# louisaslett/PhaseType

Measured on NVIDIA B200. Metric: path_draws_per_sec, higher is better.
Workload: dtype f64

## Files before the change

### phasetype_b200/csrc/k_mhrs.cu

```cuda
#include <cooperative_groups.h>
#include "engine_internal.h"
#include "pht_philox.h"

namespace cg = cooperative_groups;

#ifndef MHRS_THREADS
#define MHRS_THREADS 256
#endif
#define MHRS_WARPS (MHRS_THREADS / 32)
#ifndef MHRS_MIN_BLOCKS
#define MHRS_MIN_BLOCKS 4
#endif
#ifndef MHRS_TAIL_MIN_BLOCKS
#define MHRS_TAIL_MIN_BLOCKS 3
#endif
#ifndef MHRS_NOINLINE_COLD
#define MHRS_COLD static __device__ __forceinline__
#else
#define MHRS_COLD static __device__ __noinline__
#endif
#define GUIDE_BITS 8
#define GUIDE (1 << GUIDE_BITS)
#ifndef END_CAP
#define END_CAP 32u
#endif
#ifndef MHRS_REPLAY_MIN_BLOCKS
#define MHRS_REPLAY_MIN_BLOCKS 4
#endif
#ifndef REPLAY_REFILL_MIN
#define REPLAY_REFILL_MIN 16
#endif
#ifndef EV_MIN
#define EV_MIN 8u
#endif
#ifndef EV_WAIT
#define EV_WAIT 16u
#endif
#ifndef PREFETCH_MIN
#define PREFETCH_MIN 8
#endif
#ifndef TAIL_CH
#define TAIL_CH 256u
#endif
#ifndef TAIL_BATCH
#define TAIL_BATCH 1u
#endif
#ifndef TAIL_LATE_P
#define TAIL_LATE_P 1024u
#endif
#ifndef TAIL_LATE_GROWTH
#define TAIL_LATE_GROWTH 4u
#endif
#ifndef DRAIN_LANES
#define DRAIN_LANES 32
#endif
#ifndef TAIL_K0
#define TAIL_K0 512u
#endif
#define TAIL_KMAX (1u << 24)
#ifndef TAIL_GROWTH
#define TAIL_GROWTH 2u
#endif
#ifndef FOUND_PERIOD
#define FOUND_PERIOD 8u
#endif
#define POOL_MIN 32u
#ifndef POOL_MAX
#define POOL_MAX 256u
#endif
#define FOUND_NONE 0xFFFFFFFFFFFFFFFFull
#define T52_NEVER (1ull << 52)
#define LOWBITS (1u << 20)
#define XBAR_TIMEOUT_NS 4000000000ull

#define RF_PROP 2u
#define RF_OFF 4u
#define RF_SKIP 8u

template <int NC>
struct MhrsSmem {
    static constexpr int R = NC + 1;
    unsigned long long thr[R * R];
    double cum[R * R];
    double scale[NC];
    double s[NC];
    double inv_smax;
    unsigned long long zlo[NC];
    long long zhi[NC];
    unsigned int Nacc[NC * NC];
    unsigned int Bacc[NC];
    float A[R + 3];
    unsigned int paths_done;
    unsigned int scan[MHRS_WARPS + 1];
    uint32_t pctr[MHRS_WARPS];
    float pf_yf[MHRS_THREADS]; uint32_t pf_og[MHRS_THREADS], pf_pos[MHRS_THREADS];
    uint32_t mh_cur_a[MHRS_THREADS], mh_misc[MHRS_THREADS];
    unsigned char guide[R * GUIDE];
};

__device__ __forceinline__ unsigned long long gtimer() {
    unsigned long long t; asm volatile("mov.u64 %0, %globaltimer;" : "=l"(t)); return t;
}
__device__ __forceinline__ float lg2_approx(float x) {
    float r; asm("lg2.approx.ftz.f32 %0, %1;" : "=f"(r) : "f"(x)); return r;
}

__device__ __forceinline__ pht_u32x4 philox_block(uint32_t c0, uint32_t c1, uint32_t c2, uint32_t c3, const SweepParams &p) {
    PHT_PHILOX_ROUND(p.rk.k[0], p.rk.k[1])   PHT_PHILOX_ROUND(p.rk.k[2], p.rk.k[3])   PHT_PHILOX_ROUND(p.rk.k[4], p.rk.k[5])
    PHT_PHILOX_ROUND(p.rk.k[6], p.rk.k[7])   PHT_PHILOX_ROUND(p.rk.k[8], p.rk.k[9])   PHT_PHILOX_ROUND(p.rk.k[10], p.rk.k[11])
    PHT_PHILOX_ROUND(p.rk.k[12], p.rk.k[13]) PHT_PHILOX_ROUND(p.rk.k[14], p.rk.k[15]) PHT_PHILOX_ROUND(p.rk.k[16], p.rk.k[17])
    PHT_PHILOX_ROUND(p.rk.k[18], p.rk.k[19])
    pht_u32x4 out; out.v[0] = c0; out.v[1] = c1; out.v[2] = c2; out.v[3] = c3;
    return out;
}

struct Walk {
    double t, spare;
    uint32_t spare_hi, a, b;
    int j;
    bool odd, fresh;
};
struct Rec { double lastt; int B; long out_idx; double *z2; };

__device__ __forceinline__ void walk_begin(Walk &w, uint32_t a, bool off, uint32_t og, const SweepParams &p, uint32_t iter) {
    w.a = a; w.fresh = true; w.b = 0; w.odd = false; w.t = 0.0; w.j = 0; w.spare = 0.0; w.spare_hi = 0u;
    if (off) {
        pht_u32x4 r = philox_block(0u, a, og, iter, p);
        w.spare = pht_u01(r.v[2], r.v[3]); w.spare_hi = r.v[3]; w.odd = true; w.b = 1;
    }
}

__device__ __forceinline__ double log_unit(double x) { return pht_log_core(pht_d2u(x), 0); }

template <bool RECORD, int NC>
__device__ __forceinline__ bool walk_step(Walk &w, double y, bool cens, uint32_t og, const SweepParams &p, MhrsSmem<NC> &sm,
                                          uint32_t iter, int n, Rec &rec) {
    constexpr int R = NC + 1;
    pht_u32x4 r = philox_block(w.b, w.a, og, iter, p);
    w.b++;
    const double f = pht_u01(r.v[0], r.v[1]), g = pht_u01(r.v[2], r.v[3]);
    const double uA = w.odd ? w.spare : f;
    const uint32_t hiA = w.odd ? w.spare_hi : r.v[1];
    const double uB = w.odd ? f : g;
    w.spare = g; w.spare_hi = r.v[3];
    const bool fresh = w.fresh;
    const int row = fresh ? n : w.j;
    const int last = fresh ? n - 1 : n;
    const double *c = sm.cum + row * R;
    int k = sm.guide[row * GUIDE + (hiA >> (32 - GUIDE_BITS))] & 0x7f;
    while (k < last && c[k] < uA) k++;
    const bool cont = (k < n) && (w.t < y || cens);
    const bool ended = !fresh && !cont;
    const bool advance = !fresh && cont;
    if (RECORD) {
        if (advance) {
            rec.z2[w.j] += w.t - rec.lastt;
            if (p.outN != nullptr) p.outN[(size_t)rec.out_idx * n * n + w.j + k * n]++;
            else atomicAdd(&sm.Nacc[w.j + k * n], 1u);
        }
        rec.lastt = fresh ? 0.0 : (advance ? w.t : rec.lastt);
        rec.B = fresh ? k : rec.B;
    }
    const double tb = fresh ? 0.0 : w.t;
    const int jn = ended ? w.j : k;
    const double tn = tb + sm.scale[jn] * (-log_unit(uB));
    w.t = ended ? w.t : tn;
    w.j = jn;
    w.fresh = false;
    return ended;
}

template <int NC, bool IV = false>
MHRS_COLD uint32_t exact_attempt(uint32_t a, bool off, double y, bool cens, uint32_t og, const SweepParams &p,
                                                      MhrsSmem<NC> &sm, uint32_t iter, int n, uint32_t smask, double u = 0.0) {
    Walk w; Rec norec; norec.lastt = 0.0; norec.B = 0; norec.out_idx = 0; norec.z2 = nullptr;
    walk_begin(w, a, off, og, p, iter);
    unsigned st = 1;
    while (!walk_step<false>(w, y, cens, og, p, sm, iter, n, norec)) st++;
    bool ok = (w.t >= y) && ((smask >> w.j) & 1u);
    if constexpr (IV) ok = ok && w.t <= u;
// ... 143 lines not shown
    f.row = absd ? f.row : k;
    return end;
}

template <bool IV>
__device__ __forceinline__ bool fast_survives(const Fast &f, const typename ObsOf<IV>::T &o) {
    bool s = f.t - o.yn > f.dacc;
    if constexpr (IV) s = s && -(f.t - o.un) > f.dacc;
    return s;
}

template <int NC>
__device__ __forceinline__ void build_tables(const SweepParams &p, MhrsSmem<NC> &sm, int n, const ModelLayout &ML) {
    constexpr int R = NC + 1;
    const int tid = threadIdx.x;
    double smax = 0.0;
    for (int i = 0; i < n; i++) { const double sc = p.model[ML.scale + i]; smax = (sc > smax) ? sc : smax; }
    const double inv_smax = 1.0 / smax;
    for (int i = tid; i < n; i += MHRS_THREADS) {
        const double sc = p.model[ML.scale + i];
        sm.scale[i] = sc; sm.s[i] = p.model[ML.s + i]; sm.zlo[i] = 0ull; sm.zhi[i] = 0; sm.Bacc[i] = 0u;
        sm.A[i] = (float)((-0.69314718055994530942 * sc) * inv_smax);
    }
    if (tid == 0) { sm.A[n] = 0.0f; sm.inv_smax = inv_smax; }
    for (int i = tid; i < n * n; i += MHRS_THREADS) sm.Nacc[i] = 0u;
    for (int e = tid; e < R * R; e += MHRS_THREADS) {
        const int row = e / R, k = e % R;
        unsigned long long t52 = T52_NEVER; double c = 0.0;
        if (row <= n && k <= n) {
            c = p.model[ML.cum + row * (n + 1) + k];
            const int last = (row == n) ? n - 1 : n;
            if (k < last && c < 1.0) {
                if (!(c > 0.0)) t52 = 0ull;
                else {
                    const unsigned long long xf = (unsigned long long)(c * 4503599627370496.0);
                    const double u = pht_u2d(0x3ff0000000000000ULL | xf) - 0.99999999999999988898;
                    t52 = (u > c) ? xf : xf + 1ull;
                }
            }
        }
        sm.thr[e] = t52; sm.cum[e] = c;
    }
    if (tid == 0) sm.paths_done = 0u;
    __syncthreads();
    for (int e = tid; e < (n + 1) * GUIDE; e += MHRS_THREADS) {
        const int row = e / GUIDE, b = e % GUIDE, last = (row == n) ? n - 1 : n;
        const double floor_u = (double)b * (1.0 / GUIDE);
        int k = 0;
        while (k < last && sm.cum[row * R + k] <= floor_u) k++;
        const bool pure = sm.thr[row * R + k] >= ((unsigned long long)(b + 1) << (52 - GUIDE_BITS));
        sm.guide[e] = (unsigned char)(k | (pure ? 0x80 : 0));
    }
    __syncthreads();
}

__device__ __forceinline__ uint32_t pack_flags(bool have_cur, bool cur_off, bool off, bool cens, int cur_pre, uint32_t kprop) {
    return (have_cur ? TI_HAVE : 0u) | (cur_off ? TI_CUROFF : 0u) | (off ? TI_OFF : 0u) | (cens ? TI_CENS : 0u) |
           ((uint32_t)(cur_pre & 0xff) << 8) | (kprop << 16);
}

__device__ __forceinline__ void peer_barrier(cg::grid_group &grid, const SweepParams &p, unsigned long long epoch) {
    const unsigned long long t_in = (blockIdx.x == 0 && threadIdx.x == 0) ? gtimer() : 0ull;
    __threadfence_system();
    grid.sync();
    if (blockIdx.x == 0) {
        const int t = threadIdx.x;
        if (t < (int)p.obs_world && p.state->xdead == 0u) {
            volatile unsigned long long *mine = &p.xpeer[t]->flags[p.obs_rank];
            __threadfence_system();
            *mine = epoch;
            __threadfence_system();
            volatile unsigned long long *theirs = &p.xw->flags[t];
            const unsigned long long t0 = gtimer();
            while (*theirs < epoch) {
                if (gtimer() - t0 > XBAR_TIMEOUT_NS) { p.state->xdead = 1u; atomicOr(&p.state->error, 64); break; }
            }
            __threadfence_system();
        }
    }
    grid.sync();
    if (blockIdx.x == 0 && threadIdx.x == 0) atomicAdd(&p.state->counters[PHT_CNT_NS_XWAIT], gtimer() - t_in);
}

struct TailView {
    TailItem *items; const uint32_t *pend; unsigned long long *found; uint32_t P, K;
    bool global; uint32_t parity;
    const double *u;
};

template <int NC, bool IV = false>
__device__ __forceinline__ void tail_search(const TailView &tv, const SweepParams &p, MhrsSmem<NC> &sm, uint32_t iter, int n,
                                            uint32_t smask, uint32_t nwarps,
                                            unsigned &c_jumps, unsigned &c_attempts) {
    const unsigned FULL = 0xffffffffu; const int lane = threadIdx.x & 31;
    const uint32_t W = tv.global ? p.obs_world : 1u;
    const uint32_t Pl = (tv.P + W - 1u) / W;
    const unsigned long long total_units = (unsigned long long)Pl * tv.K;
    Fast f; fast_begin(f, 0u, n);
    typename ObsOf<IV>::T mo; obs_set(mo, 0.0f, 0u, false); obs_set_u(mo, 0.0f);
    uint32_t my_item = 0xFFFFFFFFu; bool active = false;
    unsigned steps = 0;
    uint32_t *ctr = &sm.pctr[threadIdx.x >> 5];
    if (lane == 0) *ctr = 0u;
    __syncwarp();
    unsigned long long u_next = 0, u_end = 0, last_base = 0, remaining = total_units;
    bool out_of_units = false, finished = false;
    uint32_t item = 0, og = 0, a_first = 0, pool_end = 0; float yf = 0.0f, uf = 0.0f; bool cens = false, first_off = false;
    while (!finished) {
        bool want_exact = false, exact_off = false, survived = false; int kend = 0;
#define TAIL_GRAB() do { \
            const uint32_t na_ = atomicAdd(ctr, 1u); \
            if (na_ < pool_end) { \
                my_item = item; obs_set(mo, yf, og, cens); obs_set_u(mo, uf); fast_begin(f, na_, n); \
                 \
                if (first_off && na_ == a_first) { want_exact = true; exact_off = true; active = false; } else active = true; \
            } else active = false; \
        } while (0)
        for (;;) {
            const unsigned idle = __ballot_sync(FULL, !active);
            if (idle) {
                uint32_t cur = *reinterpret_cast<volatile uint32_t *>(ctr);
                if (cur >= pool_end && !out_of_units) {
                    bool have = false; uint32_t pstart = 0u;
                    while (!have) {
                        if (u_next >= u_end) {
                            remaining = total_units > last_base ? total_units - last_base : 0ull;
                            unsigned long long want = remaining / (2ull * (unsigned long long)nwarps);
                            want = want < POOL_MIN ? POOL_MIN : (want > POOL_MAX ? POOL_MAX : want);
                            unsigned long long base = 0;
                            if (lane == 0) base = atomicAdd(&p.state->unit_counter, want);
                            base = __shfl_sync(FULL, base, 0);
                            last_base = base;
                            if (base >= total_units) { out_of_units = true; break; }
                            u_next = base; u_end = base + want < total_units ? base + want : total_units;
                        }
                        const unsigned long long chunk = u_next / TAIL_CH;
                        const unsigned long long chunk_end_u = (chunk + 1ull) * TAIL_CH;
                        const unsigned long long stop = u_end < chunk_end_u ? u_end : chunk_end_u;
                        const uint32_t q = (uint32_t)(chunk / Pl), col = (uint32_t)(chunk % Pl);
                        const uint32_t o = tv.global ? col * W + (p.obs_rank + W - q % W) % W : col;
                        const uint32_t within = (uint32_t)(u_next - chunk * TAIL_CH), len = (uint32_t)(stop - u_next);
                        u_next = stop;
                        if (o >= tv.P) continue;
                        const uint32_t it_idx = tv.pend[o];
                        const TailItem it = tv.items[it_idx];
                        if (it.flags & TI_FIN) continue;
                        pstart = it.a + q * TAIL_CH + within;
                        if ((__ldcg(&tv.found[it_idx]) >> 8) >= (unsigned long long)pstart) {
                            have = true;
                            item = it_idx; a_first = it.a; first_off = (it.flags & TI_OFF) != 0u;
                            pool_end = pstart + len;
                            yf = (float)(it.y * sm.inv_smax); cens = (it.flags & TI_CENS) != 0u; og = it.og;
                            if constexpr (IV) uf = (float)(tv.u[it_idx] * sm.inv_smax);
                        }
                    }
                    if (have) {
                        __syncwarp();
                        if (lane == 0) *ctr = pstart;
                        __syncwarp();
                        cur = pstart;
                    }
                }
                if (cur >= pool_end) { if (idle == FULL) { finished = true; break; } }
                else if (!active) TAIL_GRAB();
            }
            if (((++steps) & (FOUND_PERIOD - 1u)) == 0u) {
                unsigned long long fw = 0;
                if (lane == 0) fw = __ldcg(&tv.found[item]);
                fw = __shfl_sync(FULL, fw, 0);
                if (fw != FOUND_NONE) {
                    const uint32_t fa = (uint32_t)(fw >> 8);
                    pool_end = pool_end < fa ? pool_end : fa;
                    if (my_item == item && active && f.a > fa) { active = false; c_jumps += f.b; }
                }
            }
            __syncwarp();
            if (active) {
                bool fail;
                if (fast_step<NC, IV>(f, mo, IV ? mo.c0y : bound_c0(mo.yn), p, sm, iter, n, fail)) {
                    const bool surv = !fail && fast_survives<IV>(f, mo);
                    if (surv && !((smask >> f.row) & 1u)) fail = true;
                    if (fail) { c_attempts++; c_jumps += f.b; TAIL_GRAB(); }
                    else if (surv) { c_attempts++; c_jumps += f.b; survived = true; kend = f.row; active = false; }
                    else { c_jumps += f.b; want_exact = true; active = false; }
                }
            }
            if (__any_sync(FULL, survived || want_exact)) break;
        }
#undef TAIL_GRAB
        if (finished) break;
        if (want_exact) {
            const uint32_t res = exact_attempt<NC, IV>(f.a, exact_off, tv.items[my_item].y, mo.cens, mo.og, p, sm, iter, n, smask,
                                                       upper_at<IV>(tv.u, my_item));
            c_jumps += res >> 16; c_attempts++;
            survived = res & 1u; kend = (int)((res >> 8) & 0xffu);
        }
        const unsigned smk = __ballot_sync(FULL, survived);
        if (survived) {
            const unsigned long long word = ((unsigned long long)f.a << 8) | (unsigned long long)kend;
            atomicMin(&tv.found[my_item], word);
            if (tv.global) {
                for (uint32_t r = 0; r < p.obs_world; r++)
                    if (r != p.obs_rank) atomicMin_system(&p.xpeer[r]->gfound[tv.parity][my_item], word);
                __threadfence_system();
            }
        }
        if (smk) {
            const int src = __ffs(smk) - 1;
            const uint32_t s_item = __shfl_sync(FULL, my_item, src), s_a = __shfl_sync(FULL, f.a, src);
            if (my_item == s_item && active && f.a > s_a) { active = false; c_jumps += f.b; }
            if (s_item == item) pool_end = pool_end < s_a ? pool_end : s_a;
        }
        __syncwarp();
    }
}

MHRS_COLD int tail_advance(TailItem &it, unsigned long long fword, uint32_t K, const SweepParams &p,
                                            const double *s_model, uint32_t iter, bool &failed) {
    failed = false;
    if (fword == FOUND_NONE) {
        failed = true;
        if (it.a > 0xF0000000u - K) return 2;
        it.a += K; it.flags &= ~TI_OFF;
        return 0;
    }
    const uint32_t a = (uint32_t)(fword >> 8); const int pre = (int)(fword & 0xffull);
    const bool off = (a == it.a) && (it.flags & TI_OFF);
    const bool cens = (it.flags & TI_CENS) != 0u;
    bool have_cur = it.flags & TI_HAVE; bool cur_off = it.flags & TI_CUROFF;
    int cur_pre = (int)((it.flags >> 8) & 0xffu); uint32_t kprop = it.flags >> 16;
    bool next_off = false, done;
    if (!have_cur) {
        have_cur = true; it.cur_a = a; cur_off = off; cur_pre = pre;
        done = cens || p.mhit == 0;
    } else {
        pht_u32x4 r = philox_block(0u, a + 1u, it.og, iter, p);
        const double U = pht_u01(r.v[0], r.v[1]);
        if (U < s_model[pre] / s_model[cur_pre]) { it.cur_a = a; cur_off = off; cur_pre = pre; }
        kprop++; done = (int)kprop >= p.mhit; next_off = true;
    }
    it.a = a + 1u;
    it.flags = pack_flags(have_cur, cur_off, next_off, cens, cur_pre, kprop);
    return done ? 1 : 0;
}

#define LF_RUN 1u
#define LF_HAVE 2u
#define LF_CENS 4u
#define LF_NVALID 8u
#define LF_NCENS 16u
template <int NC, bool IV = false>
__device__ __forceinline__ void lane_phase(const SweepParams &p, MhrsSmem<NC> &sm, uint32_t iter, int n, uint32_t smask,
                                           uint32_t obs_begin, uint32_t obs_end, uint32_t cap,
                                           unsigned &c_jumps, unsigned &c_attempts) {
    const unsigned FULL = 0xffffffffu;
    const int tid = threadIdx.x, lane = tid & 31;
    Fast f; fast_begin(f, 0u, n);
    typename ObsOf<IV>::T o; obs_set(o, 0.0f, 0u, false); obs_set_u(o, 0.0f);
    const double inv_smax = sm.inv_smax;
    uint32_t pos = 0, a_lim = cap, fl = 0u;
    bool dry = false;
    for (;;) {
        const unsigned empty = __ballot_sync(FULL, !(fl & LF_NVALID));
        if (!dry && __popc(empty) >= PREFETCH_MIN) {
            const unsigned cnt = __popc(empty);
            unsigned long long base = 0;
            if (lane == 0) base = (unsigned long long)obs_begin + atomicAdd(&p.state->next_obs, (unsigned long long)cnt);
            base = __shfl_sync(FULL, base, 0);
            const unsigned long long left = base < obs_end ? (unsigned long long)obs_end - base : 0ull;
            const unsigned avail = left < cnt ? (unsigned)left : cnt;
            if (avail < cnt) dry = true;
            const unsigned rank = __popc(empty & ((1u << lane) - 1u));
            if (!(fl & LF_NVALID) && rank < avail) {
                const unsigned long long q = base + rank;
                sm.pf_pos[tid] = (uint32_t)q; sm.pf_yf[tid] = (float)(p.y[q] * inv_smax);
                sm.pf_og[tid] = p.obs_rank + (p.perm ? p.perm[q] : (uint32_t)q) * p.obs_world;
                fl |= LF_NVALID | (p.cens[q] != 0 ? LF_NCENS : 0u);
            }
        }
        if (!(fl & LF_RUN) && (fl & LF_NVALID)) {
            obs_set(o, sm.pf_yf[tid], sm.pf_og[tid], (fl & LF_NCENS) != 0u); pos = sm.pf_pos[tid];
            if constexpr (IV) obs_set_u(o, (float)(p.u[pos] * inv_smax));
            fl = LF_RUN | (o.cens ? LF_CENS : 0u);
            sm.mh_cur_a[tid] = 0u; sm.mh_misc[tid] = 0u; a_lim = cap;
            fast_begin(f, 0u, n);
        }
        const unsigned running = __ballot_sync(FULL, fl & LF_RUN);
        if (running == 0u) { if (dry) break; else continue; }
        if (dry && __popc(running) <= DRAIN_LANES && a_lim != 0xFFFFFFFFu && a_lim > END_CAP) a_lim = END_CAP;
        __syncwarp();
        bool go = (fl & LF_RUN) != 0u;
        unsigned waited = 0u, ev;
        do {
#pragma unroll
            for (int h = 0; h < 2; h++) {
                if (go) {
                    bool fail;
                    const bool end = fast_step<NC, IV>(f, o, o.c0y, p, sm, iter, n, fail);
                    if (fail) { c_jumps += f.b; fast_begin(f, f.a + 1u, n); c_attempts++; }
                    go = fail ? f.a < a_lim : !end;
                }
            }
            ev = __ballot_sync(FULL, !go);
            waited += ((ev & running) != 0u) ? 2u : 0u;
        } while (ev != 0xffffffffu && (unsigned)__popc(ev & running) < EV_MIN && waited < EV_WAIT);
        const bool stopped = (fl & LF_RUN) && !go;
        bool hand = stopped && f.b == 0u, surv = false, amb = false; int k = f.row;
        if (stopped && f.b != 0u) {
            c_jumps += f.b;
            surv = fast_survives<IV>(f, o); amb = !surv;
        }
        if (amb) {
            const uint32_t res = exact_attempt<NC, IV>(f.a, false, p.y[pos], o.cens, o.og, p, sm, iter, n, ~0u, upper_at<IV>(p.u, pos));
            surv = res & 1u; k = (int)((res >> 8) & 0xffu); c_jumps += res >> 16;
            if (!surv) { fast_begin(f, f.a + 1u, n); c_attempts++; hand = f.a >= a_lim; }
        }
        if (surv && !((smask >> k) & 1u)) { surv = false; fast_begin(f, f.a + 1u, n); c_attempts++; hand = f.a >= a_lim; }
        bool this_off = false;
        while (surv) {
            c_attempts++;
            bool complete = false; uint32_t rfl = 0u, ra1 = 0u, ra2 = 0u;
            uint32_t cur_a = sm.mh_cur_a[tid], misc = sm.mh_misc[tid];
            int cur_pre = (int)(misc & 0xffu); bool cur_off = (misc >> 8) & 1u; uint32_t kprop = misc >> 16;
            if (!(fl & LF_HAVE)) {
                fl |= LF_HAVE; cur_a = f.a; cur_off = this_off; cur_pre = k;
                if (o.cens || p.mhit == 0) { complete = true; ra1 = cur_a; rfl = cur_off ? RF_OFF : 0u; }
            } else if (p.mhit == 1) {
                complete = true; ra1 = cur_a; ra2 = f.a;
                rfl = RF_PROP | ((uint32_t)cur_pre << 8) | ((uint32_t)k << 16);
            } else {
                pht_u32x4 r = philox_block(0u, f.a + 1u, o.og, iter, p);
                const double U = pht_u01(r.v[0], r.v[1]);
                if (U < sm.s[k] / sm.s[cur_pre]) { cur_a = f.a; cur_off = this_off; cur_pre = k; }
                kprop++;
                if ((int)kprop >= p.mhit) { complete = true; ra1 = cur_a; rfl = cur_off ? RF_OFF : 0u; }
            }
            sm.mh_cur_a[tid] = cur_a; sm.mh_misc[tid] = (uint32_t)cur_pre | (cur_off ? 0x100u : 0u) | (kprop << 16);
            if (complete) {
                p.recs[pos] = make_uint4(ra1, ra2, rfl, 0u);
                fl &= ~LF_RUN; surv = false;
            } else if (kprop == 0u) {
                fast_begin(f, f.a + 1u, n); surv = false;
            } else {
                const uint32_t a = f.a + 1u;
                const uint32_t res = exact_attempt<NC, IV>(a, true, p.y[pos], o.cens, o.og, p, sm, iter, n, smask, upper_at<IV>(p.u, pos));
                surv = res & 1u; k = (int)((res >> 8) & 0xffu); c_jumps += res >> 16;
                this_off = true;
                if (!surv) c_attempts++;
                fast_begin(f, surv ? a : a + 1u, n);
            }
        }
        if (hand && (fl & LF_RUN)) {
            const uint32_t idx = atomicAdd(&p.state->n_items, 1u);
            if (idx < p.item_cap) {
                const uint32_t misc = sm.mh_misc[tid];
                TailItem it; it.y = p.y[pos]; it.og = o.og; it.pos = pos; it.a = f.a; it.cur_a = sm.mh_cur_a[tid];
                it.flags = pack_flags((fl & LF_HAVE) != 0u, (misc >> 8) & 1u, false, o.cens, (int)(misc & 0xffu), misc >> 16);
                it.owner = p.obs_rank;
                p.items[idx] = it; p.found[idx] = FOUND_NONE;
                if constexpr (IV) p.item_u[idx] = p.u[pos];
                atomicAdd(&p.state->counters[PHT_CNT_DEFERRED], 1ull);
                fl &= ~LF_RUN;
            } else a_lim = 0xFFFFFFFFu;
        }
        __syncwarp();
    }
}

template <int NC>
__device__ __forceinline__ void flush_block(const SweepParams &p, MhrsSmem<NC> &sm, int n, bool stats, unsigned c_attempts, unsigned c_jumps) {
    const unsigned FULL = 0xffffffffu; const int tid = threadIdx.x;
    __syncthreads();
    if (stats) {
        unsigned long long *gN = reinterpret_cast<unsigned long long *>(p.stats);
        for (int i = tid; i < n * n; i += MHRS_THREADS) if (sm.Nacc[i]) atomicAdd(&gN[i], (unsigned long long)sm.Nacc[i]);
        for (int i = tid; i < n; i += MHRS_THREADS) {
            if (sm.Bacc[i]) atomicAdd(&gN[n * n + i], (unsigned long long)sm.Bacc[i]);
            if (sm.zlo[i]) atomicAdd(&gN[n * n + n + i], sm.zlo[i]);
            if (sm.zhi[i]) atomicAdd(&gN[n * n + 2 * n + i], (unsigned long long)sm.zhi[i]);
        }
    }
    unsigned long long w_attempts = c_attempts, w_jumps = c_jumps;
    for (int o = 16; o > 0; o >>= 1) { w_attempts += __shfl_down_sync(FULL, w_attempts, o); w_jumps += __shfl_down_sync(FULL, w_jumps, o); }
    if ((tid & 31) == 0) { atomicAdd(&p.state->counters[PHT_CNT_ATTEMPTS], w_attempts); atomicAdd(&p.state->counters[PHT_CNT_JUMPS], w_jumps); }
    if (tid == 0 && sm.paths_done) atomicAdd(&p.state->counters[PHT_CNT_PATHS], (unsigned long long)sm.paths_done);
}

template <int NC>
// ... 10 lines not shown
    const uint32_t iter = p.state->iter;
    const unsigned long long t0 = (blockIdx.x == 0 && threadIdx.x == 0) ? gtimer() : 0ull;
    build_tables(p, sm, n, ModelLayout::make(n, p.m));
    uint32_t smask;
    model_scalars(sm, n, smask);
    const bool per_obs = p.outB != nullptr;
    const uint32_t obs_begin = per_obs ? (uint32_t)p.first : 0u;
    const uint32_t obs_end = per_obs ? (uint32_t)(p.first + p.count) : (uint32_t)p.l_local;
    const uint32_t cap = p.mhrs_cap > 0 ? (uint32_t)p.mhrs_cap : 256u;
    unsigned c_attempts = 0, c_jumps = 0;
    lane_phase<NC, IV>(p, sm, iter, n, smask, obs_begin, obs_end, cap, c_jumps, c_attempts);
    flush_block(p, sm, n, false, c_attempts, c_jumps);
    if (blockIdx.x == 0 && threadIdx.x == 0) atomicAdd(&p.state->counters[PHT_CNT_NS_LANE], gtimer() - t0);
}

template <int NC, bool IV>
__global__ void __launch_bounds__(MHRS_THREADS, MHRS_TAIL_MIN_BLOCKS) k_mhrs_tail(const __grid_constant__ SweepParams p) {
    extern __shared__ __align__(16) unsigned char smem_raw[];
    cg::grid_group grid = cg::this_grid();
    MhrsSmem<NC> &sm = *reinterpret_cast<MhrsSmem<NC> *>(smem_raw);
    const int n = p.n, tid = threadIdx.x;
    const uint32_t iter = p.state->iter;
    const bool per_obs = p.outB != nullptr;
    const bool multi = p.xw != nullptr && p.obs_world > 1u && !per_obs;
    const uint32_t n_items = p.state->n_items < p.item_cap ? p.state->n_items : p.item_cap;
    if (n_items == 0u && !multi) return;
    const bool timekeeper = (blockIdx.x == 0 && tid == 0);
    unsigned long long t_mark = timekeeper ? gtimer() : 0ull;
    build_tables(p, sm, n, ModelLayout::make(n, p.m));
    uint32_t smask;
    model_scalars(sm, n, smask);
    const double *s_model = p.model + ModelLayout::make(n, p.m).s;
    unsigned c_attempts = 0, c_jumps = 0;
    const uint32_t gtid = blockIdx.x * MHRS_THREADS + tid, gsize = gridDim.x * MHRS_THREADS, nwarps = gsize / 32u;

    for (uint32_t i = gtid; i < n_items; i += gsize) p.pend0[i] = i;
    if (gtid == 0) {
        p.state->n_pend[0] = n_items; p.state->n_pend[1] = 0u; p.state->unit_counter = 0ull;
        p.state->any_fail[0] = 0u; p.state->any_fail[1] = 0u;
    }
    grid.sync();
    uint32_t K = TAIL_K0; while (K < (uint32_t)p.mhrs_cap && K < TAIL_KMAX) K *= 2u;
    uint32_t rounds = 0u, g0 = 0u, Pg = 0u; int cur = 0, gl_cur = 0; bool global = false;
    const uint32_t W = p.obs_world, me = p.obs_rank, sp = iter & 1u;
    unsigned long long epoch = multi ? p.state->xepoch : 0ull;
    for (;;) {
        const uint32_t *pend = cur ? p.pend1 : p.pend0;
        uint32_t *pend_next = cur ? p.pend0 : p.pend1;
        if (!global) {
            const uint32_t P = p.state->n_pend[cur];
            const bool leave = P == 0u || (multi && K >= p.k_switch && P <= PHT_GCAP);
            if (leave && !multi) break;
            if (leave) {
                if (timekeeper) { const unsigned long long t = gtimer(); atomicAdd(&p.state->counters[PHT_CNT_NS_TAIL], t - t_mark); t_mark = t; }
                for (uint32_t r = 0; r < W; r++) {
                    XchgWindow *dst = p.xpeer[r];
                    for (uint32_t i = gtid; i < P; i += gsize) {
                        dst->gitems[sp][me * PHT_GCAP + i] = p.items[pend[i]];
                        if constexpr (IV) dst->gitem_u[sp][me * PHT_GCAP + i] = p.item_u[pend[i]];
                    }
                    if (gtid == 0) dst->gcount[sp][me] = P;
                }
                peer_barrier(grid, p, ++epoch);
                for (uint32_t r = 0; r < W; r++) {
                    const uint32_t c = p.xw->gcount[sp][r] <= PHT_GCAP ? p.xw->gcount[sp][r] : PHT_GCAP;
                    for (uint32_t i = gtid; i < c; i += gsize) p.glist[Pg + i] = r * PHT_GCAP + i;
                    Pg += c;
                }
                if (gtid == 0) {
                    p.state->n_gpend = Pg; p.state->unit_counter = 0ull; p.state->any_fail[0] = 0u; p.state->any_fail[1] = 0u;
                    atomicAdd(&p.state->counters[PHT_CNT_GLOBAL_ITEMS], (unsigned long long)Pg);
                }
                grid.sync();
                global = true; g0 = rounds;
                K = p.k_switch > TAIL_K0 ? p.k_switch : TAIL_K0;
                continue;
            }
        } else if (Pg == 0u || p.state->xdead != 0u) break;
        const uint32_t par = (rounds - g0) & 1u;
        TailView tv;
        if (!global) { tv.items = p.items; tv.pend = pend; tv.found = p.found; tv.P = p.state->n_pend[cur]; tv.u = p.item_u; }
        else { tv.items = p.xw->gitems[sp]; tv.pend = gl_cur ? p.glist + PHT_MAX_WORLD * PHT_GCAP : p.glist; tv.found = p.xw->gfound[par]; tv.P = Pg; tv.u = p.xw->gitem_u[sp]; }
        tv.K = K; tv.global = global; tv.parity = par;
        const unsigned long long tr0 = timekeeper ? gtimer() : 0ull;
        const unsigned att0 = c_attempts, jmp0 = c_jumps;
        tail_search<NC, IV>(tv, p, sm, iter, n, smask, nwarps, c_jumps, c_attempts);
        const unsigned long long tr1 = timekeeper ? gtimer() : 0ull;
        if (rounds < PHT_ROUND_TRACE) {
            unsigned d = c_attempts - att0;
            for (int o = 16; o > 0; o >>= 1) d += __shfl_xor_sync(0xffffffffu, d, o);
            if ((tid & 31) == 0 && d) atomicAdd(&p.state->round_trace[rounds][5], (unsigned long long)d);
            unsigned dj = c_jumps - jmp0;
            for (int o = 16; o > 0; o >>= 1) dj += __shfl_xor_sync(0xffffffffu, dj, o);
            if ((tid & 31) == 0 && dj) atomicAdd(&p.state->round_trace[rounds][7], (unsigned long long)dj);
        }
        if (global) peer_barrier(grid, p, ++epoch); else grid.sync();
        const unsigned long long tr2 = timekeeper ? gtimer() : 0ull;
        for (uint32_t i = gtid; i < tv.P; i += gsize) {
            const uint32_t item = tv.pend[i];
            TailItem it = tv.items[item];
            if (it.flags & TI_FIN) continue;
            bool failed;
            if (rounds < PHT_ROUND_TRACE && (!global || it.owner == me)) {
                const unsigned long long fw = tv.found[item];
                atomicAdd(&p.state->round_trace[rounds][6], fw == FOUND_NONE ? (unsigned long long)K : (unsigned long long)((uint32_t)(fw >> 8) - it.a + 1u));
            }
            const int st = tail_advance(it, tv.found[item], K, p, s_model, iter, failed);
            tv.found[item] = FOUND_NONE;
            if (st != 0 && global) it.flags |= TI_FIN;
            tv.items[item] = it;
            const bool mine = !global || it.owner == me;
            if (st == 2 && mine) { atomicAdd(&p.state->counters[PHT_CNT_ERRORS], 1ull); atomicOr(&p.state->error, 8); }
            if (failed && st == 0) atomicOr(&p.state->any_fail[par], 1u);
            if (st != 0 && mine) p.recs[it.pos] = (st == 1) ? make_uint4(it.cur_a, 0u, (it.flags & TI_CUROFF) ? RF_OFF : 0u, 0u) : make_uint4(0u, 0u, RF_SKIP, 0u);
            if (st == 0 && !global) pend_next[atomicAdd(&p.state->n_pend[cur ^ 1], 1u)] = item;
        }
        if (gtid == 0) { if (!global) p.state->n_pend[cur] = 0u; p.state->unit_counter = 0ull; p.state->any_fail[par ^ 1u] = 0u; }
        grid.sync();
        if (global) {
            uint32_t *next_list = (gl_cur ? p.glist : p.glist + PHT_MAX_WORLD * PHT_GCAP);
            if (blockIdx.x == 0) {
                const int lane = tid & 31, warp = tid >> 5;
                uint32_t outn = 0u;
                for (uint32_t tile = 0; tile < Pg; tile += MHRS_THREADS) {
                    const uint32_t i = tile + tid;
                    uint32_t item = 0u; bool keep = false;
                    if (i < Pg) { item = tv.pend[i]; keep = !(tv.items[item].flags & TI_FIN); }
                    const unsigned bal = __ballot_sync(0xffffffffu, keep);
                    if (lane == 0) sm.scan[warp] = __popc(bal);
                    __syncthreads();
                    uint32_t off = 0u, tot = 0u;
                    for (int w2 = 0; w2 < MHRS_WARPS; w2++) { const uint32_t c = sm.scan[w2]; off += (w2 < warp) ? c : 0u; tot += c; }
                    if (keep) next_list[outn + off + __popc(bal & ((1u << lane) - 1u))] = item;
                    outn += tot;
                    __syncthreads();
                }
                if (tid == 0) p.state->n_gpend = outn;
            }
            grid.sync();
            Pg = p.state->n_gpend; gl_cur ^= 1;
        }
        const bool grow = p.state->any_fail[par] != 0u;
        if (timekeeper && rounds < PHT_ROUND_TRACE) {
            unsigned long long *tr = p.state->round_trace[rounds];
            tr[0] += tr1 - tr0; tr[1] += tr2 - tr1; tr[2] += gtimer() - tr2; tr[3] += tv.P; tr[4] += K;
        }
        if (!global) cur ^= 1;
        rounds++;
        if (grow && K < TAIL_KMAX) K *= ((global ? Pg : p.state->n_pend[cur]) <= TAIL_LATE_P) ? TAIL_LATE_GROWTH : TAIL_GROWTH;
        if (K > TAIL_KMAX) K = TAIL_KMAX;
    }
    if (multi && gtid == 0) { p.state->xepoch = epoch; p.state->n_pend[cur] = 0u; }
    if (timekeeper) {
        const unsigned long long t = gtimer();
        atomicAdd(&p.state->counters[global ? PHT_CNT_NS_GLOBAL : PHT_CNT_NS_TAIL], t - t_mark); t_mark = t;
    }
    if (gtid == 0) {
        atomicAdd(&p.state->counters[PHT_CNT_TAIL_ROUNDS], (unsigned long long)rounds);
        if (global) atomicAdd(&p.state->counters[PHT_CNT_GLOBAL_ROUNDS], (unsigned long long)(rounds - g0));
    }
    flush_block(p, sm, n, false, c_attempts, c_jumps);
}

template <int NC>
__global__ void __launch_bounds__(MHRS_THREADS, MHRS_REPLAY_MIN_BLOCKS) k_mhrs_replay(const __grid_constant__ SweepParams p) {
    extern __shared__ __align__(16) unsigned char smem_raw[];
    MhrsSmem<NC> &sm = *reinterpret_cast<MhrsSmem<NC> *>(smem_raw);
    const int n = p.n;
    const uint32_t iter = p.state->iter;
// ... 63 lines not shown
```

Baseline: 953.3 million.

## Restructure tail search into per-warp shared pools with range grabs and batched stepping

Rewrites the tail search so each warp keeps its work pool in shared memory, lanes grab ranges of attempts (up to TAIL_RANGE) instead of single attempts, and stepping uses a shared search_steps helper with periodic found-word polling. The goals are to cut per-attempt atomics, reduce divergence from the old one-step-at-a-time loop, and reuse the batched stepping loop from the main sampler. It also raises tail min-blocks, which adds register pressure. The added complexity risks subtle correctness issues in how early stops and pool ends are handled.

```diff
diff --git a/phasetype_b200/csrc/k_mhrs.cu b/phasetype_b200/csrc/k_mhrs.cu
--- a/phasetype_b200/csrc/k_mhrs.cu
+++ b/phasetype_b200/csrc/k_mhrs.cu
@@ -12,7 +12,7 @@
 #define MHRS_MIN_BLOCKS 4
 #endif
 #ifndef MHRS_TAIL_MIN_BLOCKS
-#define MHRS_TAIL_MIN_BLOCKS 3
+#define MHRS_TAIL_MIN_BLOCKS 4
 #endif
 #ifndef MHRS_NOINLINE_COLD
 #define MHRS_COLD static __device__ __forceinline__
@@ -42,8 +42,8 @@
 #ifndef TAIL_CH
 #define TAIL_CH 256u
 #endif
-#ifndef TAIL_BATCH
-#define TAIL_BATCH 1u
+#ifndef TAIL_RANGE
+#define TAIL_RANGE 8u
 #endif
 #ifndef TAIL_LATE_P
 #define TAIL_LATE_P 1024u
@@ -61,8 +61,8 @@
 #ifndef TAIL_GROWTH
 #define TAIL_GROWTH 2u
 #endif
-#ifndef FOUND_PERIOD
-#define FOUND_PERIOD 8u
+#ifndef POLL_VOTES
+#define POLL_VOTES 8u
 #endif
 #define POOL_MIN 32u
 #ifndef POOL_MAX
@@ -76,6 +76,20 @@
 #define RF_PROP 2u
 #define RF_OFF 4u
 #define RF_SKIP 8u
+
+struct TailView {
+    TailItem *items; const uint32_t *pend; unsigned long long *found; uint32_t P, K;
+    bool global; uint32_t parity;
+    const double *u;
+};
+#define TP_OFF 1u
+#define TP_CENS 2u
+#define TP_OUT 4u
+struct TailPool {
+    unsigned long long u_next, u_end, last_base;
+    uint32_t item, end, a_first, og, flags, range;
+    float yf, uf;
+};
 
 template <int NC>
 struct MhrsSmem {
@@ -96,6 +110,8 @@
     float pf_yf[MHRS_THREADS]; uint32_t pf_og[MHRS_THREADS], pf_pos[MHRS_THREADS];
     uint32_t mh_cur_a[MHRS_THREADS], mh_misc[MHRS_THREADS];
     unsigned char guide[R * GUIDE];
+    TailView tv;
+    TailPool pool[MHRS_WARPS];
 };
 
 __device__ __forceinline__ unsigned long long gtimer() {
@@ -405,136 +421,164 @@
     if (blockIdx.x == 0 && threadIdx.x == 0) atomicAdd(&p.state->counters[PHT_CNT_NS_XWAIT], gtimer() - t_in);
 }
 
-struct TailView {
-    TailItem *items; const uint32_t *pend; unsigned long long *found; uint32_t P, K;
-    bool global; uint32_t parity;
-    const double *u;
-};
-
-template <int NC, bool IV = false>
-__device__ __forceinline__ void tail_search(const TailView &tv, const SweepParams &p, MhrsSmem<NC> &sm, uint32_t iter, int n,
-                                            uint32_t smask, uint32_t nwarps,
-                                            unsigned &c_jumps, unsigned &c_attempts) {
-    const unsigned FULL = 0xffffffffu; const int lane = threadIdx.x & 31;
+template <int NC, bool IV, bool POLL>
+__device__ __forceinline__ bool search_steps(Fast &f, const typename ObsOf<IV>::T &o, uint32_t a_lim, bool go, unsigned running,
+                                             const SweepParams &p, const MhrsSmem<NC> &sm, uint32_t iter, int n,
+                                             const unsigned long long *found, uint32_t item, unsigned &votes,
+                                             unsigned &c_jumps, unsigned &c_attempts) {
+    unsigned waited = 0u, ev;
+    do {
+#pragma unroll
+        for (int h = 0; h < 2; h++) {
+            if (go) {
+                bool fail;
+                const bool end = fast_step<NC, IV>(f, o, o.c0y, p, sm, iter, n, fail);
+                if (fail) { c_jumps += f.b; fast_begin(f, f.a + 1u, n); c_attempts++; }
+                go = fail ? f.a < a_lim : !end;
+            }
+        }
+        if (POLL && ((++votes) & (POLL_VOTES - 1u)) == 0u && go) {
+            if (f.a > (uint32_t)(__ldcg(&found[item]) >> 8)) { c_jumps += f.b; fast_begin(f, a_lim, n); go = false; }
+        }
+        ev = __ballot_sync(0xffffffffu, !go);
+        waited += ((ev & running) != 0u) ? 2u : 0u;
+        if (POLL && __any_sync(0xffffffffu, !go && f.b != 0u)) waited = EV_WAIT;
+    } while (ev != 0xffffffffu && (unsigned)__popc(ev & running) < EV_MIN && waited < EV_WAIT);
+    return go;
+}
+
+
+template <int NC, bool IV>
+__device__ __forceinline__ void tail_pool(const SweepParams &p, MhrsSmem<NC> &sm, uint32_t nwarps) {
+    const unsigned FULL = 0xffffffffu; const int lane = threadIdx.x & 31, warp = threadIdx.x >> 5;
+    const TailView &tv = sm.tv;
+    TailPool &tp = sm.pool[warp];
     const uint32_t W = tv.global ? p.obs_world : 1u;
     const uint32_t Pl = (tv.P + W - 1u) / W;
     const unsigned long long total_units = (unsigned long long)Pl * tv.K;
+    unsigned long long u_next = tp.u_next, u_end = tp.u_end, last_base = tp.last_base, remaining;
+    bool have = false;
+    while (!have) {
+        if (u_next >= u_end) {
+            remaining = total_units > last_base ? total_units - last_base : 0ull;
+            unsigned long long want = remaining / (2ull * (unsigned long long)nwarps);
+            want = want < POOL_MIN ? POOL_MIN : (want > POOL_MAX ? POOL_MAX : want);
+            unsigned long long base = 0;
+            if (lane == 0) base = atomicAdd(&p.state->unit_counter, want);
+            base = __shfl_sync(FULL, base, 0);
+            last_base = base;
+            if (base >= total_units) break;
+            u_next = base; u_end = base + want < total_units ? base + want : total_units;
+        }
+        const unsigned long long chunk = u_next / TAIL_CH;
+        const unsigned long long chunk_end_u = (chunk + 1ull) * TAIL_CH;
+        const unsigned long long stop = u_end < chunk_end_u ? u_end : chunk_end_u;
+        const uint32_t q = (uint32_t)(chunk / Pl), col = (uint32_t)(chunk % Pl);
+        const uint32_t o = tv.global ? col * W + (p.obs_rank + W - q % W) % W : col;
+        const uint32_t within = (uint32_t)(u_next - chunk * TAIL_CH), len = (uint32_t)(stop - u_next);
+        u_next = stop;
+        if (o >= tv.P) continue;
+        const uint32_t it_idx = tv.pend[o];
+        const TailItem it = tv.items[it_idx];
+        if (it.flags & TI_FIN) continue;
+        const uint32_t pstart = it.a + q * TAIL_CH + within;
+        if ((__ldcg(&tv.found[it_idx]) >> 8) >= (unsigned long long)pstart) {
+            have = true;
+            if (lane == 0) {
+                tp.item = it_idx; tp.a_first = it.a; tp.end = pstart + len; tp.og = it.og;
+                tp.range = len / 32u < 1u ? 1u : (len / 32u > TAIL_RANGE ? TAIL_RANGE : len / 32u);
+                tp.yf = (float)(it.y * sm.inv_smax);
+                if constexpr (IV) tp.uf = (float)(tv.u[it_idx] * sm.inv_smax);
+                tp.flags = ((it.flags & TI_OFF) ? TP_OFF : 0u) | ((it.flags & TI_CENS) ? TP_CENS : 0u);
+                sm.pctr[warp] = pstart;
+            }
+        }
+    }
+    if (lane == 0) {
+        tp.u_next = u_next; tp.u_end = u_end; tp.last_base = last_base;
+        if (!have) tp.flags |= TP_OUT;
+    }
+    __syncwarp();
+}
+
+__device__ __forceinline__ void tail_found(const TailView &tv, TailPool &tp, const SweepParams &p, uint32_t item, uint32_t a, int k) {
+    const unsigned long long word = ((unsigned long long)a << 8) | (unsigned long long)k;
+    atomicMin(&tv.found[item], word);
+    if (tv.global) {
+        for (uint32_t r = 0; r < p.obs_world; r++)
+            if (r != p.obs_rank) atomicMin_system(&p.xpeer[r]->gfound[tv.parity][item], word);
+        __threadfence_system();
+    }
+    if (item == tp.item) atomicMin(&tp.end, a);
+}
+
+template <int NC, bool IV = false>
+__device__ __forceinline__ void tail_search(const SweepParams &p, MhrsSmem<NC> &sm, uint32_t iter, int n,
+                                            uint32_t smask, uint32_t nwarps,
+                                            unsigned &c_jumps, unsigned &c_attempts) {
+    const unsigned FULL = 0xffffffffu; const int lane = threadIdx.x & 31, warp = threadIdx.x >> 5;
+    const TailView &tv = sm.tv;
+    TailPool &tp = sm.pool[warp];
+    uint32_t *ctr = &sm.pctr[warp];
+    volatile uint32_t *vctr = ctr, *vend = &tp.end;
+    if (lane == 0) { *ctr = 0u; tp.end = 0u; tp.item = 0xFFFFFFFFu; tp.flags = 0u; tp.u_next = 0ull; tp.u_end = 0ull; tp.last_base = 0ull; }
+    __syncwarp();
     Fast f; fast_begin(f, 0u, n);
-    typename ObsOf<IV>::T mo; obs_set(mo, 0.0f, 0u, false); obs_set_u(mo, 0.0f);
-    uint32_t my_item = 0xFFFFFFFFu; bool active = false;
-    unsigned steps = 0;
-    uint32_t *ctr = &sm.pctr[threadIdx.x >> 5];
-    if (lane == 0) *ctr = 0u;
-    __syncwarp();
-    unsigned long long u_next = 0, u_end = 0, last_base = 0, remaining = total_units;
-    bool out_of_units = false, finished = false;
-    uint32_t item = 0, og = 0, a_first = 0, pool_end = 0; float yf = 0.0f, uf = 0.0f; bool cens = false, first_off = false;
-    while (!finished) {
-        bool want_exact = false, exact_off = false, survived = false; int kend = 0;
-#define TAIL_GRAB() do { \
-            const uint32_t na_ = atomicAdd(ctr, 1u); \
-            if (na_ < pool_end) { \
-                my_item = item; obs_set(mo, yf, og, cens); obs_set_u(mo, uf); fast_begin(f, na_, n); \
-                 \
-                if (first_off && na_ == a_first) { want_exact = true; exact_off = true; active = false; } else active = true; \
-            } else active = false; \
-        } while (0)
+    typename ObsOf<IV>::T o; obs_set(o, 0.0f, 0u, false); obs_set_u(o, 0.0f);
+    uint32_t item = 0u, a_lim = 0u;
+    unsigned votes = 0u;
+    bool go = false;
+    for (;;) {
+        bool surv = false; int k = f.row;
+        if (!go && f.b != 0u) {
+            c_jumps += f.b;
+            surv = fast_survives<IV>(f, o);
+            if (!surv) {
+                const uint32_t res = exact_attempt<NC, IV>(f.a, false, tv.items[item].y, o.cens, o.og, p, sm, iter, n, ~0u,
+                                                           upper_at<IV>(tv.u, item));
+                surv = res & 1u; k = (int)((res >> 8) & 0xffu); c_jumps += res >> 16;
+                if (!surv) { fast_begin(f, f.a + 1u, n); c_attempts++; }
+            }
+            if (surv && !((smask >> k) & 1u)) { surv = false; fast_begin(f, f.a + 1u, n); c_attempts++; }
+        }
+        const unsigned smk = __ballot_sync(FULL, surv);
+        if (smk) {
+            if (surv) { c_attempts++; tail_found(tv, tp, p, item, f.a, k); }
+            const int src = __ffs(smk) - 1;
+            const uint32_t s_item = __shfl_sync(FULL, item, src), s_a = __shfl_sync(FULL, f.a, src);
+            if (surv || (item == s_item && f.a > s_a && f.a < a_lim)) { if (!surv) c_jumps += f.b; fast_begin(f, a_lim, n); }
+            __syncwarp();
+        }
         for (;;) {
-            const unsigned idle = __ballot_sync(FULL, !active);
-            if (idle) {
-                uint32_t cur = *reinterpret_cast<volatile uint32_t *>(ctr);
-                if (cur >= pool_end && !out_of_units) {
-                    bool have = false; uint32_t pstart = 0u;
-                    while (!have) {
-                        if (u_next >= u_end) {
-                            remaining = total_units > last_base ? total_units - last_base : 0ull;
-                            unsigned long long want = remaining / (2ull * (unsigned long long)nwarps);
-                            want = want < POOL_MIN ? POOL_MIN : (want > POOL_MAX ? POOL_MAX : want);
-                            unsigned long long base = 0;
-                            if (lane == 0) base = atomicAdd(&p.state->unit_counter, want);
-                            base = __shfl_sync(FULL, base, 0);
-                            last_base = base;
-                            if (base >= total_units) { out_of_units = true; break; }
-                            u_next = base; u_end = base + want < total_units ? base + want : total_units;
-                        }
-                        const unsigned long long chunk = u_next / TAIL_CH;
-                        const unsigned long long chunk_end_u = (chunk + 1ull) * TAIL_CH;
-                        const unsigned long long stop = u_end < chunk_end_u ? u_end : chunk_end_u;
-                        const uint32_t q = (uint32_t)(chunk / Pl), col = (uint32_t)(chunk % Pl);
-                        const uint32_t o = tv.global ? col * W + (p.obs_rank + W - q % W) % W : col;
-                        const uint32_t within = (uint32_t)(u_next - chunk * TAIL_CH), len = (uint32_t)(stop - u_next);
-                        u_next = stop;
-                        if (o >= tv.P) continue;
-                        const uint32_t it_idx = tv.pend[o];
-                        const TailItem it = tv.items[it_idx];
-                        if (it.flags & TI_FIN) continue;
-                        pstart = it.a + q * TAIL_CH + within;
-                        if ((__ldcg(&tv.found[it_idx]) >> 8) >= (unsigned long long)pstart) {
-                            have = true;
-                            item = it_idx; a_first = it.a; first_off = (it.flags & TI_OFF) != 0u;
-                            pool_end = pstart + len;
-                            yf = (float)(it.y * sm.inv_smax); cens = (it.flags & TI_CENS) != 0u; og = it.og;
-                            if constexpr (IV) uf = (float)(tv.u[it_idx] * sm.inv_smax);
-                        }
-                    }
-                    if (have) {
-                        __syncwarp();
-                        if (lane == 0) *ctr = pstart;
-                        __syncwarp();
-                        cur = pstart;
+            if (__ballot_sync(FULL, !(f.a < a_lim)) == 0u) break;
+            __syncwarp();
+            if (!(*vctr < *vend)) {
+                if (tp.flags & TP_OUT) break;
+                tail_pool<NC, IV>(p, sm, nwarps);
+                continue;
+            }
+            if (lane == 0) { const uint32_t fa = (uint32_t)(__ldcg(&tv.found[tp.item]) >> 8); if (fa < tp.end) tp.end = fa; }
+            __syncwarp();
+            if (!(f.a < a_lim) && *vctr < *vend) {
+                const uint32_t na = atomicAdd(ctr, tp.range), pe = *vend;
+                if (na < pe) {
+                    item = tp.item; a_lim = na + tp.range < pe ? na + tp.range : pe;
+                    obs_set(o, tp.yf, tp.og, (tp.flags & TP_CENS) != 0u); obs_set_u(o, tp.uf);
+                    fast_begin(f, na, n);
+                    if (na == tp.a_first && (tp.flags & TP_OFF)) {
+                        const uint32_t res = exact_attempt<NC, IV>(na, true, tv.items[item].y, o.cens, o.og, p, sm, iter, n, smask,
+                                                                   upper_at<IV>(tv.u, item));
+                        c_jumps += res >> 16; c_attempts++;
+                        if (res & 1u) { tail_found(tv, tp, p, item, na, (int)((res >> 8) & 0xffu)); a_lim = na + 1u; }
+                        fast_begin(f, na + 1u, n);
                     }
                 }
-                if (cur >= pool_end) { if (idle == FULL) { finished = true; break; } }
-                else if (!active) TAIL_GRAB();
-            }
-            if (((++steps) & (FOUND_PERIOD - 1u)) == 0u) {
-                unsigned long long fw = 0;
-                if (lane == 0) fw = __ldcg(&tv.found[item]);
-                fw = __shfl_sync(FULL, fw, 0);
-                if (fw != FOUND_NONE) {
-                    const uint32_t fa = (uint32_t)(fw >> 8);
-                    pool_end = pool_end < fa ? pool_end : fa;
-                    if (my_item == item && active && f.a > fa) { active = false; c_jumps += f.b; }
-                }
-            }
-            __syncwarp();
-            if (active) {
-                bool fail;
-                if (fast_step<NC, IV>(f, mo, IV ? mo.c0y : bound_c0(mo.yn), p, sm, iter, n, fail)) {
-                    const bool surv = !fail && fast_survives<IV>(f, mo);
-                    if (surv && !((smask >> f.row) & 1u)) fail = true;
-                    if (fail) { c_attempts++; c_jumps += f.b; TAIL_GRAB(); }
-                    else if (surv) { c_attempts++; c_jumps += f.b; survived = true; kend = f.row; active = false; }
-                    else { c_jumps += f.b; want_exact = true; active = false; }
-                }
-            }
-            if (__any_sync(FULL, survived || want_exact)) break;
-        }
-#undef TAIL_GRAB
-        if (finished) break;
-        if (want_exact) {
-            const uint32_t res = exact_attempt<NC, IV>(f.a, exact_off, tv.items[my_item].y, mo.cens, mo.og, p, sm, iter, n, smask,
-                                                       upper_at<IV>(tv.u, my_item));
-            c_jumps += res >> 16; c_attempts++;
-            survived = res & 1u; kend = (int)((res >> 8) & 0xffu);
-        }
-        const unsigned smk = __ballot_sync(FULL, survived);
-        if (survived) {
-            const unsigned long long word = ((unsigned long long)f.a << 8) | (unsigned long long)kend;
-            atomicMin(&tv.found[my_item], word);
-            if (tv.global) {
-                for (uint32_t r = 0; r < p.obs_world; r++)
-                    if (r != p.obs_rank) atomicMin_system(&p.xpeer[r]->gfound[tv.parity][my_item], word);
-                __threadfence_system();
-            }
-        }
-        if (smk) {
-            const int src = __ffs(smk) - 1;
-            const uint32_t s_item = __shfl_sync(FULL, my_item, src), s_a = __shfl_sync(FULL, f.a, src);
-            if (my_item == s_item && active && f.a > s_a) { active = false; c_jumps += f.b; }
-            if (s_item == item) pool_end = pool_end < s_a ? pool_end : s_a;
-        }
-        __syncwarp();
+            }
+        }
+        go = f.a < a_lim;
+        const unsigned running = __ballot_sync(FULL, go);
+        if (running == 0u) break;
+        go = search_steps<NC, IV, true>(f, o, a_lim, go, running, p, sm, iter, n, tv.found, item, votes, c_jumps, c_attempts);
     }
 }
 
@@ -612,21 +656,9 @@
         if (running == 0u) { if (dry) break; else continue; }
         if (dry && __popc(running) <= DRAIN_LANES && a_lim != 0xFFFFFFFFu && a_lim > END_CAP) a_lim = END_CAP;
         __syncwarp();
-        bool go = (fl & LF_RUN) != 0u;
-        unsigned waited = 0u, ev;
-        do {
-#pragma unroll
-            for (int h = 0; h < 2; h++) {
-                if (go) {
-                    bool fail;
-                    const bool end = fast_step<NC, IV>(f, o, o.c0y, p, sm, iter, n, fail);
-                    if (fail) { c_jumps += f.b; fast_begin(f, f.a + 1u, n); c_attempts++; }
-                    go = fail ? f.a < a_lim : !end;
-                }
-            }
-            ev = __ballot_sync(FULL, !go);
-            waited += ((ev & running) != 0u) ? 2u : 0u;
-        } while (ev != 0xffffffffu && (unsigned)__popc(ev & running) < EV_MIN && waited < EV_WAIT);
+        unsigned votes = 0u;
+        const bool go = search_steps<NC, IV, false>(f, o, a_lim, (fl & LF_RUN) != 0u, running, p, sm, iter, n, nullptr, 0u, votes,
+                                                    c_jumps, c_attempts);
         const bool stopped = (fl & LF_RUN) && !go;
         bool hand = stopped && f.b == 0u, surv = false, amb = false; int k = f.row;
         if (stopped && f.b != 0u) {
@@ -803,9 +835,11 @@
         if (!global) { tv.items = p.items; tv.pend = pend; tv.found = p.found; tv.P = p.state->n_pend[cur]; tv.u = p.item_u; }
         else { tv.items = p.xw->gitems[sp]; tv.pend = gl_cur ? p.glist + PHT_MAX_WORLD * PHT_GCAP : p.glist; tv.found = p.xw->gfound[par]; tv.P = Pg; tv.u = p.xw->gitem_u[sp]; }
         tv.K = K; tv.global = global; tv.parity = par;
+        if (tid == 0) sm.tv = tv;
+        __syncthreads();
         const unsigned long long tr0 = timekeeper ? gtimer() : 0ull;
         const unsigned att0 = c_attempts, jmp0 = c_jumps;
-        tail_search<NC, IV>(tv, p, sm, iter, n, smask, nwarps, c_jumps, c_attempts);
+        tail_search<NC, IV>(p, sm, iter, n, smask, nwarps, c_jumps, c_attempts);
         const unsigned long long tr1 = timekeeper ? gtimer() : 0ull;
         if (rounds < PHT_ROUND_TRACE) {
             unsigned d = c_attempts - att0;
```

New measurement: 949.7 million (median of 6 runs). About the same (-0.4%).
